# jacketsj/expANN

Measured on AMD Instinct MI355X. Metric: queries/sec at recall@10=1.0 (exact brute force), 1Mxd128 fp32, k=10, higher is better.
Workload: dtype f32; 1 GPU; brute_force_engine L2 N=1000000 d=128 fp32, 10000 batched queries, k=10 (BASELINE configs[1]); n=1000000, d=128, m=10000, k=10, metric=l2, launch=one process, one GPU, devices_visible=1, comm_ranks=0

## Files before the change

### expann_amd/csrc/expann_hip.hip

```cpp
#include "../../include/expann_hip.h"

#include <hip/hip_runtime.h>

#include <algorithm>
#include <cmath>
#include <cstdio>
#include <cstdlib>
#include <cstring>
#include <iterator>
#include <memory>
#include <mutex>
#include <string>
#include <vector>

#include "bf_append.hpp"
#include "bf_remove.hpp"
#include "bf_options.hpp"
#include "bf_plan.hpp"
#include "host_common.hpp"
#include "scan_f32.hpp"
#include "scan_gemm_bf16.hpp"
#include "scan_gemm_f16.hpp"
#include "scan_gemm_f16x.hpp"
#include "scan_gemm_f16kx.hpp"
#include "scan_direct_f16.hpp"
#include "scan_gemm_i8.hpp"
#include "scan_gemm_i8q.hpp"
#include "scan_gemm_i8w.hpp"
#include "scan_gemm_w8.hpp"
#include "scan_gemm_kl.hpp"
#include "scan_int8.hpp"
#include "scan_int8_any.hpp"
#include "filter_rows.hpp"
#include "scan_groups.hpp"
#include "append_rows.hpp"
#include "remove_rows.hpp"
#include "score_ids.hpp"
#include "select.hpp"
#include "select_range.hpp"

using namespace expann;

namespace expann {
thread_local std::string g_create_error;
}

namespace {

static_assert(kMaxK == kMaxCap / 2, "the bound on k: a candidate list holds at least 2k keys");
constexpr size_t kMaxQueriesPerPass = 32768;
constexpr int kEventPairs = 64;
constexpr uint32_t kAsyncRing = 256;
constexpr uint32_t kRingWords = 10, kRingScale = 8, kRingMark = 9;
constexpr size_t kFlagCopyBytes = sizeof(uint32_t) * 7;
constexpr uint32_t kFilterListCap = kMaxCap;

struct Level {
	uint32_t n_groups_sel;
	uint32_t group_stride;
	uint32_t classmin_blocks = 0;
	uint32_t list_rows = 0;
	uint32_t list_step = 1;
};

}


struct Config : Options {
	int dim = 0, dtype = 0, metric = 0, device = 0;
	size_t elem = 4;
	size_t q_elem = 4;
	int int_mode = -1;
	bool strict_u8 = false;
};

struct Rows {
	std::vector<unsigned char> staging;
	size_t n_staged = 0;
	MaybeOwnedPtr d_base;
	size_t n = 0;
	size_t capacity = 0;
	size_t reserved = 0;
	uint64_t id_offset = 0;
};

struct HandleDeleter {
	void operator()(expann_index* h) const { expann_destroy(h); }
};
struct U8Shadow {
	int u8_exact = 0;
	DevPtr<void> d_base_u8;
	std::unique_ptr<expann_index, HandleDeleter> u8_shadow;
};

struct F16Copy {
	DevPtr<float> d_bnmax;
	DevPtr<void> d_base_f16;
	DevPtr<float> d_bnorm_f16;
	DevPtr<float> d_bns_f16;
	float f16_scale = 0.0f;
	float f16_maxabs = 0.0f;
	size_t f16_n_pad = 0;
	size_t f16_tb = 0;
	size_t f16_rows_alloc = 0;
};
struct OtherCopies : U8Shadow {
	DevPtr<float> d_bnorm_bf;
	DevPtr<void> d_base_split;
	DevPtr<void> d_base_i8f;
	DevPtr<int> d_bp_i8f;
	DevPtr<float> d_rw_i8f;
// ... 811 lines not shown
	*tiles_big = big;
	*n_big = nb;
	*tiles_small = small;
	*n_small = ns;
	return true;
}

constexpr double kSpecFailTarget = 0.01;
double spec_fail_share(size_t k, double f, uint32_t j) {
	if (j == 0)
		return 1.0;
	if (k <= 1 || j > k - 1)
		return 0.0;
	f = std::min(1.0, std::max(0.0, f));
	const double n = (double)(k - 1);
	double term = std::pow(1.0 - f, n), below = 0.0;
	for (uint32_t i = 0; i < j; ++i) {
		below += term;
		term = f < 1.0 ? term * (n - i) / (i + 1.0) * f / (1.0 - f) : 0.0;
	}
	return f < 1.0 ? std::max(0.0, 1.0 - below) : 1.0;
}
uint32_t spec_rank_auto(size_t k, double f) {
	for (uint32_t j = 1; j < k; ++j)
		if (spec_fail_share(k, f, j) <= kSpecFailTarget)
			return j;
	return (uint32_t)k;
}
uint32_t spec_redo_slots(size_t m) {
	const size_t want = (size_t)std::ceil(4.0 * kSpecFailTarget * (double)m);
	return (uint32_t)(std::max<size_t>(1, (want + kF16TQ - 1) / kF16TQ) * kF16TQ);
}

uint32_t sample_frac_for(const expann_index* h, size_t k) {
	if (h->opt_sample_frac > 0)
		return (uint32_t)h->opt_sample_frac;
	const double expo = float_rows(h) ? 0.3 : 0.5;
	const double bytes = (double)h->n * (double)h->dim * (float_rows(h) ? 2.0 : 1.0);
	double size = (bytes >= 8 * 2.56e8 && k <= 32) ? std::min(3.0, std::pow(bytes / 2.56e8, 0.3)) : 1.0;
	if (float_rows(h) && k > 32)
		size = 0.75 * std::pow(std::max(1.0, bytes / 3.2e8), 0.25);
	const double f = 16.0 * std::pow(10.0 / (double)std::max<size_t>(1, k), expo) * size;
	return (uint32_t)std::min(48.0, std::max(4.0, std::round(f)));
}

using GemmI8qFn = void (*)(GemmI8qParams);
using SelfI8AnyFn = void (*)(const void*, uint32_t, int*, uint32_t);
using ThetaI8AnyFn = void (*)(const void*, uint32_t, const float*, int*, int*, uint32_t);
struct GemmI8qVariant {
	int d, mode;
	GemmI8qFn scan, sample;
	SelfI8Fn self;
	ThetaI8Fn theta;
	const char* name;
	int dq;
	int lds, threads, wg_per_cu;
	void (*scan_w)(GemmI8wParams) = nullptr;
	int lds_w = 0, threads_w = 0, wg_per_cu_w = 0;
	void (*sample_w)(GemmI8wParams) = nullptr;
	int tb = kF16TB;
	SelfI8AnyFn self_any = nullptr;
	ThetaI8AnyFn theta_any = nullptr;
};
#define GEMM_I8X_P(D, DQ, MODE, L2F, MN) {D, MODE, scan_gemm_w8_kernel<I8Elem, DQ, false, D, L2F>, \
	scan_gemm_w8_kernel<I8Elem, DQ, true, D, L2F>, row_self_i8_kernel<D, MODE>, query_theta_i8_kernel<D, MODE>, \
	"scan_gemm_i8x<" #DQ "," MN ">", DQ, gemm_i8q_lds_bytes<DQ>(), I8qGeom<DQ>::THREADS, I8qGeom<DQ>::WG_PER_CU}
const GemmI8qVariant kGemmI8x[] = {
    GEMM_I8X_P(768, 768, kU8L2, true, "U8L2"), GEMM_I8X_P(768, 768, kI8L2, true, "I8L2"), GEMM_I8X_P(768, 768, kI8IP, false, "I8IP"),
    GEMM_I8X_P(832, 1024, kU8L2, true, "U8L2"), GEMM_I8X_P(832, 1024, kI8L2, true, "I8L2"),
    GEMM_I8X_P(832, 1024, kI8IP, false, "I8IP"),
    GEMM_I8X_P(960, 1024, kU8L2, true, "U8L2"), GEMM_I8X_P(960, 1024, kI8L2, true, "I8L2"),
    GEMM_I8X_P(960, 1024, kI8IP, false, "I8IP"),
    GEMM_I8X_P(896, 1024, kU8L2, true, "U8L2"), GEMM_I8X_P(896, 1024, kI8L2, true, "I8L2"),
    GEMM_I8X_P(896, 1024, kI8IP, false, "I8IP")};
#undef GEMM_I8X_P
#define GEMM_I8W(D, MODE, L2F, MN) {D, MODE, nullptr, nullptr, row_self_i8_kernel<D, MODE>, \
	query_theta_i8_kernel<D, MODE>, "scan_gemm_i8w<" #D "," MN ">", D, gemm_i8q_lds_bytes<D>(), kF16Threads, \
	I8wGeom<D>::WG_PER_CU, scan_gemm_i8w_kernel<D, L2F>, gemm_i8w_lds_bytes<D>(), kF16Threads, I8wGeom<D>::WG_PER_CU, \
	scan_gemm_i8w_kernel<D, L2F, true>}
const GemmI8qVariant kGemmI8w[] = {
    GEMM_I8W(128, kU8L2, true, "U8L2"), GEMM_I8W(128, kI8L2, true, "I8L2"), GEMM_I8W(128, kI8IP, false, "I8IP"),
    GEMM_I8W(256, kU8L2, true, "U8L2"), GEMM_I8W(256, kI8L2, true, "I8L2"), GEMM_I8W(256, kI8IP, false, "I8IP")};
const GemmI8qVariant kGemmI8F = GEMM_I8W(128, kI8L2, true, "F32L2");
void (*const kGemmI8FRedo)(GemmI8wParams) = scan_gemm_i8w_kernel<128, true, false, true>;
#undef GEMM_I8W
#define GEMM_I8KL(MODE, MN) {0, MODE, nullptr, nullptr, nullptr, nullptr, "scan_gemm_i8kl<" MN ">", 0, kKlLds, kF16Threads, 1, \
	scan_gemm_kl_kernel<I8Elem, false>, kKlLds, kF16Threads, 1, scan_gemm_kl_kernel<I8Elem, true>, kKlTB, \
	row_self_i8_any_kernel<MODE>, query_theta_i8_any_kernel<MODE>}
const GemmI8qVariant kGemmI8KL[] = {GEMM_I8KL(kU8L2, "U8L2"), GEMM_I8KL(kI8L2, "I8L2"), GEMM_I8KL(kI8IP, "I8IP")};
#undef GEMM_I8KL
constexpr int kRetryGeneric = -1000;
constexpr int kStrictReject = -1001;

const GemmI8qVariant* find_gemm_i8q(ScanFamily f, int d, int mode) {
	for (const auto& v : kGemmI8w)
		if (f == ScanFamily::kI8qW && v.d == d && v.mode == mode)
			return &v;
	for (const auto& v : kGemmI8x)
		if (f == ScanFamily::kI8qX && v.d == d && v.mode == mode)
			return &v;
	for (const auto& v : kGemmI8KL)
		if (f == ScanFamily::kI8qKL && v.mode == mode)
			return &v;
	return nullptr;
}

static_assert(kI8MinRows == 2 * 256 * kF16TB, "bf_plan.hpp: two 256-tile chunks of the int8 hit-log forms");
bool plan_tables_match() {
	bool ok = kGemmF16XDbg[0].d == kF16DbgDim && kGemmI8F.d == kI8fDim;
	auto all = [&ok](const auto& tab, size_t listed, auto in) {
		size_t hits = 0;
		for (const auto& v : tab)
			hits += in(v) ? 1 : 0;
		ok = ok && hits == std::size(tab) && hits == listed;
	};
	const auto mfma_mode = [](int mode) { return mode == kU8L2 || mode == kI8L2 || mode == kI8IP; };
	all(kScanF32, 2 * count_tiles(kScanF32Tiles, std::size(kScanF32Tiles)),
	    [](const ScanVariant& v) { return has_tile(tiles_of(kScanF32Tiles, v.d), v.tq); });
	all(kScanF32Any, 2 * count_tiles(&kScanF32AnyTiles, 1), [](const ScanVariant& v) { return has_tile(&kScanF32AnyTiles, v.tq); });
	all(kScanI8, 4 * count_tiles(kScanI8Tiles, std::size(kScanI8Tiles)) + count_tiles(kScanI16Tiles, std::size(kScanI16Tiles)),
	    [](const ScanI8Variant& v) {
		    return has_tile(v.mode == kI16L2Ref ? tiles_of(kScanI16Tiles, v.d) : tiles_of(kScanI8Tiles, v.d), v.tq);
	    });
	all(kScanI8Any, 4 * count_tiles(&kScanI8AnyTiles, 1), [](const ScanI8Variant& v) { return has_tile(&kScanI8AnyTiles, v.tq); });
	all(kDirectF16, count_tiles(kDirectF16Tiles, std::size(kDirectF16Tiles)),
	    [](const DirectF16Variant& v) { return has_tile(tiles_of(kDirectF16Tiles, v.d), v.tq); });
	all(kGemmF16X, std::size(kF16XDims) + std::size(kF16YDims) + std::size(kF16KXDims), [](const GemmF16Variant& v) {
		return (has_dim(kF16XDims, v.d) && v.scan_redo) || has_dim(kF16YDims, v.d) || has_dim(kF16KXDims, v.d);
	});
	all(kGemmBf16, std::size(kBf16Dims), [](const GemmBf16Variant& v) { return has_dim(kBf16Dims, v.d); });
	all(kGemmI8, 3 * std::size(kGemmI8Dims), [&](const GemmI8Variant& v) { return has_dim(kGemmI8Dims, v.d) && mfma_mode(v.mode); });
	all(kGemmI8w, 3 * std::size(kI8qWDims), [&](const GemmI8qVariant& v) { return has_dim(kI8qWDims, v.d) && mfma_mode(v.mode); });
	all(kGemmI8x, 3 * std::size(kI8qXDims), [&](const GemmI8qVariant& v) { return has_dim(kI8qXDims, v.d) && mfma_mode(v.mode); });
	all(kGemmI8KL, 3, [&](const GemmI8qVariant& v) { return v.d == 0 && mfma_mode(v.mode); });
	return ok;
}

constexpr double kI8fClipRms = 5.5;
constexpr double kI8fTrimEnergy = 1.0 / 16.0;
constexpr double kI8fListRatio = 2.8;
constexpr double kI8fBreakEvenRatio = 3.4;
uint64_t i8f_cand_limit(const expann_index* h, size_t m, size_t k, uint32_t spec_j = 0) {
	const double rank = spec_j ? (double)spec_j : (double)k;
	return (uint64_t)(kI8fBreakEvenRatio * 1.2 * rank * sample_frac_for(h, k) * (double)m);
}

int ensure_i8f(expann_index* h, hipStream_t st) {
	if (h->i8f_state != 0)
		return EXPANN_OK;
	const size_t nv = h->n * (size_t)h->dim;
	DevBuf tmp;
	HIP_TRY(h, tmp.alloc(16));
	HIP_TRY(h, hipMemsetAsync(tmp.p, 0, 16, st));
	hipLaunchKernelGGL(i8f_stats_kernel, dim3(2048), dim3(kBlock), 0, st, (const float*)h->d_base, nv, tmp.as<double>(),
	                   reinterpret_cast<uint32_t*>(tmp.as<double>() + 1));
	unsigned char hb[16];
	float bnmax = 0.0f;
	HIP_TRY(h, hipMemcpyAsync(hb, tmp.p, 16, hipMemcpyDeviceToHost, st));
	HIP_TRY(h, hipMemcpyAsync(&bnmax, h->d_bnmax + 2, sizeof(float), hipMemcpyDeviceToHost, st));
	HIP_TRY(h, hipStreamSynchronize(st));
	double sumsq;
	float maxabs;
	std::memcpy(&sumsq, hb, 8);
	std::memcpy(&maxabs, hb + 8, 4);
	double rms = std::sqrt(sumsq / (double)nv);
	float clip = (float)std::min<double>(maxabs, kI8fClipRms * rms);
	if (maxabs > clip && std::isfinite(clip) && clip > 0.0f) {
// ... 1087 lines not shown
	sel.bn_max = h->d_bnmax ? h->d_bnmax + (gvf ? 2 : (gvb ? 1 : 0)) : nullptr;
	sel.qnrm = (use_gemm && gvf) ? h->d_qnrm : nullptr;
	if (use_i8f) {
		sel.prune_eps = 0.0f;
		sel.prune_abs = 0.0f;
		sel.row_w = h->d_rw_i8f;
		sel.q_w = h->d_i8f_q + 2 * h->i8f_q_m;
		if (h->opt_rerank_rounds != 1) {
			sel.tau_f = spec_j ? (const float*)h->d_tau_s : (const float*)h->d_tau[levels.size() & 1];
			sel.inv_2s2 = h->i8f.inv_2s2;
		}
	}
	rerank_counted = false;
	if (last && sel.rerank_base && h->opt_rerank_stats) {
		HIP_TRY(h, grow_ws(h, h->d_rerank, 16 + sizeof(uint32_t) * m));
		HIP_TRY(h, hipMemsetAsync(h->d_rerank, 0, 16 + sizeof(uint32_t) * m, st));
		sel.rerank_cnt = reinterpret_cast<uint32_t*>(h->d_rerank.as<unsigned char>() + 16);
		rerank_counted = true;
	}
	sel.overflow = h->d_overflow;
	if (last && spec_j) {
		const RedoWs ws(redo_slots, h->dim, cap);
		sel.spec_tau = h->d_tau_s;
		sel.redo_word = h->d_overflow + 3;
		sel.redo_list = reinterpret_cast<uint32_t*>(h->d_redo.as<unsigned char>() + ws.list);
		sel.redo_cap = redo_slots;
		sel.redo_bound = reinterpret_cast<float*>(h->d_redo.as<unsigned char>() + ws.bound);
	}
	const bool sum_counts = last && sel.cand_cnt && (h->profiling || use_i8f);
	if (m > 64 && sel.rerank_base && sel.cand_cnt) {
		const uint32_t sj = last ? spec_j : 0u;
		const double expect = (use_i8f ? kI8fListRatio : 1.0) * 1.2 * (sj ? (double)sj : (double)k) * sample_frac_for(h, k);
		const int rs = launch_select(h, sel, m, cap, st, select_longest_list(expect, sj), sum_counts);
		if (rs != EXPANN_OK)
			return rs;
	} else {
		if (sum_counts)
			hipLaunchKernelGGL(sum_u32_kernel, dim3(1), dim3(1024), 0, st, sel.cand_cnt, (uint32_t)m, h->d_total);
		if (m <= 64)
			sel.wave0_short = 1;
		hipLaunchKernelGGL(select_topk_fn(h, sel), dim3((uint32_t)m), dim3(kBlock), sizeof(uint64_t) * cap + 16, st, sel);
		HIP_TRY(h, hipGetLastError());
	}
	if (last && spec_j)
		return run_redo(use_i8f);
	return EXPANN_OK;
}

int SearchPass::run_redo(bool use_i8f) {
	const RedoWs ws(redo_slots, h->dim, cap);
	unsigned char* const b = h->d_redo.as<unsigned char>();
	uint32_t* const word = h->d_overflow + 3;
	const uint32_t R = redo_slots;
	RedoCompactParams cp{};
	cp.word = word;
	cp.list = reinterpret_cast<const uint32_t*>(b + ws.list);
	cp.n_slots = R;
	cp.row_bytes = (uint32_t)h->dim * 2;
	cp.q16 = h->d_q_split;
	cp.rq16 = b + ws.q16;
	cp.qnrm = h->d_qnrm;
	cp.r_qnrm = reinterpret_cast<float*>(b + ws.qnrm);
	cp.tau = h->d_tau[levels.size() & 1];
	cp.bound = h->opt_redo_bound ? reinterpret_cast<const float*>(b + ws.bound) : nullptr;
	cp.qscale = (ip && h->opt_ip_rescale) ? h->d_qscale.as<const float>() : nullptr;
	cp.eps = gemm_f16_filter_eps(h->dim);
	cp.abs_coef = std::ldexp(1.0f, -24) / h->f16_scale * std::sqrt((float)h->dim);
	cp.mul = 0.5f * h->f16_scale * h->f16_scale;
	cp.ip = ip ? 1 : 0;
	cp.r_theta = reinterpret_cast<float*>(b + ws.theta);
	cp.r_cnt = reinterpret_cast<uint32_t*>(b + ws.cnt);
	if (use_i8f) {
		cp.q8 = h->d_q8f;
		cp.rq8 = b + ws.q8;
		cp.i8_aq = h->d_i8f_q;
		cp.i8_wq_in = h->d_i8f_q + h->i8f_q_m;
		cp.r_thp = reinterpret_cast<int*>(b + ws.thp);
		cp.r_wq = reinterpret_cast<float*>(b + ws.wq);
		cp.r_tau = reinterpret_cast<float*>(b + ws.tau);
		cp.i8_inv_2s2 = h->i8f.inv_2s2;
	}
	hipLaunchKernelGGL(redo_compact_kernel, dim3(R / (kBlock / 64)), dim3(kBlock), 0, st, cp);

	const uint32_t nt = (uint32_t)((h->n + kF16TB - 1) / kF16TB);
	const uint32_t nqt = R / kF16TQ;
	const uint32_t wg_per_cu = use_i8f ? (uint32_t)kGemmI8F.wg_per_cu_w : (uint32_t)gvf->wg_per_cu;
	uint32_t chunks = pick_row_chunks(nt, 1, wg_per_cu * (uint32_t)cus, 4.0, 8, 2048, 0, nullptr);
	chunks = std::min<uint32_t>(chunks, (uint32_t)(h->log_cnt_n / (4 * (size_t)nqt)));
	if (chunks == 0 || !h->d_log)
		return h->fail(EXPANN_ERR_HIP, "redo pass: the main scan left no hit logs");
	const uint32_t tpb = (nt + chunks - 1) / chunks;
	chunks = (nt + tpb - 1) / tpb;
	const uint32_t n_logs = chunks * nqt * 4;
	const uint32_t log_cap = (uint32_t)std::min<size_t>(1u << 16, h->log_bytes / ((size_t)n_logs * 16));
	GatherLogParams gp{};
	gp.log = h->d_log.as<const uint4>();
	gp.log_cnt = h->d_log_cnt.as<const uint32_t>();
	gp.log_cap = log_cap;
	gp.n_chunks = chunks;
	gp.n_qtiles = nqt;
	gp.m = R;
	gp.cand_cnt = cp.r_cnt;
	gp.cand = reinterpret_cast<uint64_t*>(b + ws.cand);
	gp.cap = cap;
	gp.live_q = word;
	if (use_i8f) {
		GemmI8wParams wp{};
		wp.q.base = h->d_base_i8f;
		wp.q.bp = h->d_bp_i8f;
		wp.q.n_rows = (uint32_t)h->n;
		wp.q.n_tiles_sel = nt;
		wp.q.tile_stride = 1;
		wp.q.tile_run = 1;
		wp.q.tiles_per_block = tpb;
		wp.q.n_qtiles = nqt;
		wp.q.queries = cp.rq8;
		wp.q.thp = cp.r_thp;
		wp.q.m = R;
		wp.q.cand_cnt = gp.cand_cnt;
		wp.q.cand = gp.cand;
		wp.q.cap = cap;
		wp.q.live_q = word;
		wp.log = h->d_log.as<uint4>();
		wp.log_cnt = h->d_log_cnt;
		wp.log_cap = log_cap;
		wp.lost = h->d_overflow;
		hipLaunchKernelGGL(kGemmI8FRedo, dim3(chunks * nqt), dim3((uint32_t)kGemmI8F.threads_w), kGemmI8F.lds_w, st, wp);
		gp.i_thp = cp.r_thp;
		gp.i_bias = h->d_bp_i8f;
		gp.i_rw = h->d_rw_i8f;
		gp.i_mode = 3;
	} else {
		GemmF16Params fp{};
		fp.base_f16 = h->d_base_f16;
		fp.bnorm = h->bnorm_f16();
		fp.n_rows = (uint32_t)h->n;
		fp.n_tiles_sel = nt;
		fp.tile_stride = 1;
		fp.tile_run = 1;
		fp.tiles_per_block = tpb;
		fp.n_qtiles = nqt;
		fp.queries_f16 = cp.rq16;
		fp.theta = cp.r_theta;
		fp.two_inv_s2 = (ip ? 1.0f : 2.0f) / (h->f16_scale * h->f16_scale);
		fp.m = R;
		fp.cand_cnt = gp.cand_cnt;
		fp.cand = gp.cand;
		fp.cap = cap;
		fp.ksteps = (uint32_t)f16_ld(h->dim) / 32;
		fp.log = h->d_log.as<uint4>();
		fp.log_cnt = h->d_log_cnt;
		fp.log_cap = log_cap;
		fp.lost = h->d_overflow;
		fp.live_q = word;
		hipLaunchKernelGGL(gvf->scan_redo, dim3(chunks * nqt), dim3((uint32_t)gvf->threads), gvf->lds, st, fp);
		gp.theta = cp.r_theta;
		gp.key_mul = fp.two_inv_s2;
	}
	const uint32_t want = std::max<uint32_t>(1, (1024 + nqt * 4 - 1) / (nqt * 4));
	gp.chunks_per_block = std::max<uint32_t>(1, (chunks + want - 1) / want);
	gp.n_groups = (chunks + gp.chunks_per_block - 1) / gp.chunks_per_block;
	hipLaunchKernelGGL(gather_logs_kernel, dim3(nqt * 4 * gp.n_groups), dim3(kBlock), 0, st, gp);

	SelectParams sel{};
	sel.cand = gp.cand;
	sel.cand_cnt = gp.cand_cnt;
	sel.cap = cap;
	sel.k = (uint32_t)k;
	sel.id_offset = h->id_offset;
	sel.out_ids = d_ids;
	sel.out_dists = d_dists;
	sel.rerank_base = (const float*)h->d_base;
	sel.rerank_queries = (const float*)d_queries;
	sel.dim = (uint32_t)h->dim;
	sel.metric_ip = ip ? 1u : 0u;
	const float pr = ip ? 1.0f : 2.0f;
	sel.bn_max = h->d_bnmax + 2;
	sel.qnrm = cp.r_qnrm;
	if (use_i8f) {
		sel.row_w = h->d_rw_i8f;
		sel.q_w = cp.r_wq;
		if (h->opt_rerank_rounds != 1) {
			sel.tau_f = cp.r_tau;
			sel.inv_2s2 = h->i8f.inv_2s2;
		}
	} else {
		sel.prune_eps = pr * gemm_f16_filter_eps(h->dim);
		sel.prune_abs = pr * std::ldexp(1.0f, -24) / h->f16_scale * std::sqrt((float)h->dim);
	}
	sel.overflow = word;
	sel.wave0_short = 1;
	sel.slot_map = cp.list;
	sel.live_slots = word;
	sel.redo_cand = h->d_overflow + 6;
	if (rerank_counted)
		sel.rerank_cnt = reinterpret_cast<uint32_t*>(h->d_rerank.as<unsigned char>() + 16);
	hipLaunchKernelGGL(select_topk_fn(h, sel), dim3(R), dim3(kBlock), sizeof(uint64_t) * cap + 16, st, sel);
	HIP_TRY(h, hipGetLastError());
	return EXPANN_OK;
}

int SearchPass::check(int attempt, Next* next) {
	*next = kDone;
	uint64_t reranked = 0;
	if (rerank_counted) {
		unsigned long long* const total = h->d_rerank.as<unsigned long long>();
		hipLaunchKernelGGL(sum_u32_kernel, dim3(1), dim3(1024), 0, st, reinterpret_cast<const uint32_t*>(total + 2),
		                   (uint32_t)m, total);
		unsigned long long v = 0;
		HIP_TRY(h, hipMemcpyAsync(&v, total, sizeof(v), hipMemcpyDeviceToHost, st));
		HIP_TRY(h, hipStreamSynchronize(st));
		reranked = v;
	}
	if (defer_flags(h, st, attempt)) {
		h->stat_rerank_rows += reranked;
		float sc = gvf ? h->f16_scale : 0.0f;
		uint32_t* const slot = h->h_flag_ring + kRingWords * (h->async_pending - 1);
		std::memcpy(&slot[kRingScale], &sc, sizeof(float));
		if (i8f_ran && h->opt_i8_filter == 1)
			slot[kRingMark] = 0x80000000u | (uint32_t)std::min<uint64_t>(i8f_cand_limit(h, m, k, spec_j), 0x3FFFFFFFu);
		if (spec_j)
			slot[kRingMark] |= 0x40000000u;
		return EXPANN_OK;
	}
	HIP_TRY(h, hipMemcpyAsync(h->h_flags, h->d_overflow, kFlagCopyBytes, hipMemcpyDeviceToHost, st));
	HIP_TRY(h, hipStreamSynchronize(st));
	unsigned long long tot;
	std::memcpy(&tot, h->h_flags + 4, sizeof(tot));
	h->prof.candidates = tot;
	if (i8f_ran && h->opt_i8_filter == 1 && tot > i8f_cand_limit(h, m, k, spec_j))
		h->i8f_state = 2;
	if (std::getenv("EXPANN_DEBUG_LISTS")) {
		std::vector<uint32_t> cnt(m);
		HIP_TRY(h, hipMemcpy(cnt.data(), h->d_cnt, sizeof(uint32_t) * m, hipMemcpyDeviceToHost));
		std::sort(cnt.begin(), cnt.end());
		std::fprintf(stderr, "[lists] attempt %d cap %u: min %u median %u p90 %u p99 %u max %u, overflow flag %u\n", attempt, cap,
		             cnt.front(), cnt[m / 2], cnt[m * 9 / 10], cnt[m * 99 / 100], cnt.back(), h->h_flags[0]);
	}
	if (gvf) {
		float qmax;
		std::memcpy(&qmax, &h->h_flags[2], sizeof(float));
		if (!(qmax * h->f16_scale <= 60000.0f)) {
			learned.no_f16 = true;
			h->prof.retries++;
			*next = kRestart;
			return EXPANN_OK;
		}
	}
	if (h->strict_u8 && (h->h_flags[1] != 0 || h->h_flags[3] != 0))
// ... 193 lines not shown
		}
	} else {
		g_create_error = "unknown dtype";
		return EXPANN_ERR_INVALID_ARG;
	}
	if (int_mode >= 0 && dim % 64 != 0) {
		g_create_error = "8-bit rows need dim % 64 == 0 (src/distance.h:29-53, antitopo_engine.h:726)";
		return EXPANN_ERR_INVALID_ARG;
	}
	if (int_mode >= 0 && int_mode != kI16L2Ref && dim > kMaxAnyDim) {
		g_create_error = "unsupported dim " + std::to_string(dim) + ": 8-bit rows take dim <= " +
		                 std::to_string(kMaxAnyDim);
		return EXPANN_ERR_UNSUPPORTED;
	}
	int ndev = expann_device_count();
	if (ndev <= 0) {
		g_create_error = "no HIP device visible: libexpann_hip has no CPU fallback";
		return EXPANN_ERR_NO_DEVICE;
	}
	if (device < 0 || device >= ndev) {
		g_create_error = "device index out of range";
		return EXPANN_ERR_INVALID_ARG;
	}
	PlanIndex px;
	px.dtype = dtype;
	px.int_mode = int_mode;
	px.dim = dim;
	static const bool tables_match = plan_tables_match();
	if (!tables_match) {
		g_create_error = "internal: bf_plan.hpp does not list the compiled scan kernels";
		return EXPANN_ERR_UNSUPPORTED;
	}
	if (!direct_tile(px, 1)) {
		g_create_error = "unsupported dim " + std::to_string(dim) +
		                 " (built: f32 any multiple of 16 up to 4096; 8-bit any multiple of 64 up to 4096; int16 64,128)";
		return EXPANN_ERR_UNSUPPORTED;
	}
	std::unique_ptr<expann_index, HandleDeleter> h(new expann_index());
	h->dim = dim;
	h->dtype = dtype;
	h->metric = metric;
	h->device = device;
	h->elem = (dtype == EXPANN_DTYPE_F32) ? 4 : ((dtype == EXPANN_DTYPE_I16 || dtype == EXPANN_DTYPE_F16) ? 2 : 1);
	h->q_elem = (dtype == EXPANN_DTYPE_I8) ? 1 : (dtype == EXPANN_DTYPE_I16 ? 2 : 4);
	h->int_mode = int_mode;
	static_cast<Options&>(*h) = options_from_env();
	if (hipSetDevice(device) != hipSuccess || hipStreamCreate(&h->stream) != hipSuccess) {
		g_create_error = "hipSetDevice/hipStreamCreate failed";
		return EXPANN_ERR_HIP;
	}
	struct LdsNeed {
		const void* fn;
		int bytes;
		const char* label;
	};
	std::vector<LdsNeed> needs;
	const int sel_lds = (int)(sizeof(uint64_t) * kMaxCap + 16);
	needs.push_back({(const void*)select_topk_kernel<float>, sel_lds, "select_topk_kernel"});
	needs.push_back({(const void*)select_topk_kernel<_Float16>, sel_lds, "select_topk_kernel"});
	needs.push_back({(const void*)select_topk_kernel<float, true>, sel_lds, "select_topk_kernel"});
	for (const auto& v : kGemmF16X)
		if (v.d == dim) {
			needs.push_back({(const void*)v.scan, v.lds, "scan_gemm_f16x_kernel"});
			needs.push_back({(const void*)v.sample, v.lds, "scan_gemm_f16x_kernel"});
			if (v.scan_redo)
				needs.push_back({(const void*)v.scan_redo, v.lds, "scan_gemm_f16x_kernel"});
		}
	if ((dtype == EXPANN_DTYPE_F32 || dtype == EXPANN_DTYPE_F16) && f16kl_dim(dim)) {
		needs.push_back({(const void*)kGemmF16KL.scan, kGemmF16KL.lds, "scan_gemm_kl_kernel, fp16"});
		needs.push_back({(const void*)kGemmF16KL.sample, kGemmF16KL.lds, "scan_gemm_kl_kernel, fp16"});
	}
	if (kGemmF16XDbg[0].d == dim)
		needs.push_back({(const void*)kGemmF16XDbg[0].scan, kGemmF16XDbg[0].lds, "scan_gemm_f16x_kernel"});
	for (const auto& v : kGemmI8x)
		if (v.d == dim) {
			needs.push_back({(const void*)v.scan, v.lds, "scan_gemm_w8_kernel, int8"});
			needs.push_back({(const void*)v.sample, v.lds, "scan_gemm_w8_kernel, int8"});
		}
	for (const auto& v : kGemmI8w)
		if (v.d == dim) {
			needs.push_back({(const void*)v.scan_w, v.lds_w, "scan_gemm_i8w_kernel"});
			needs.push_back({(const void*)v.sample_w, v.lds_w, "scan_gemm_i8w_kernel"});
		}
	if (dim == kGemmI8F.d)
		needs.push_back({(const void*)kGemmI8FRedo, kGemmI8F.lds_w, "scan_gemm_i8w_kernel, redo instance"});
	if (any_dim_i8(dim, int_mode))
		for (const auto& v : kGemmI8KL)
			if (v.mode == int_mode) {
				needs.push_back({(const void*)v.scan_w, v.lds_w, "scan_gemm_kl_kernel, int8"});
				needs.push_back({(const void*)v.sample_w, v.lds_w, "scan_gemm_kl_kernel, int8"});
			}
	for (const auto& v : kGemmBf16)
		if (v.d == dim)
			needs.push_back({(const void*)v.scan, 2 * kGemmTB * dim * (int)sizeof(float), "scan_gemm_bf16x3_kernel"});
	for (const auto& v : kGemmI8)
		if (v.d == dim && v.mode == int_mode)
			needs.push_back({(const void*)v.scan, 2 * gemm_i8_tb(dim) * dim, "scan_gemm_i8_kernel"});
	for (const LdsNeed& need : needs)
		if (hipFuncSetAttribute(need.fn, hipFuncAttributeMaxDynamicSharedMemorySize, need.bytes) != hipSuccess) {
			g_create_error = std::string("hipFuncSetAttribute(") + need.label + ") failed";
			return EXPANN_ERR_HIP;
		}
	*out = h.release();
	return EXPANN_OK;
}

void expann_destroy(expann_index* h) {
	if (!h)
		return;
	hipSetDevice(h->device);
	if (h->stream) hipStreamSynchronize(h->stream);
	if (h->side_stream) hipStreamSynchronize(h->side_stream);
	delete h;
}

const char* expann_last_error(const expann_index* h) {
	return h ? h->err.c_str() : g_create_error.c_str();
}

int expann_add(expann_index* h, const void* rows, size_t n) {
	if (!h)
		return EXPANN_ERR_INVALID_ARG;
	if (!rows && n)
		return h->fail(EXPANN_ERR_INVALID_ARG, "rows == NULL");
	if (h->d_base)
		return h->fail(EXPANN_ERR_INVALID_ARG, "index already built");
	const size_t bytes = n * (size_t)h->dim * h->elem;
	const unsigned char* src = static_cast<const unsigned char*>(rows);
	h->staging.insert(h->staging.end(), src, src + bytes);
	h->n_staged += n;
	return EXPANN_OK;
}

int expann_build(expann_index* h) {
	if (!h)
		return EXPANN_ERR_INVALID_ARG;
	if (h->d_base)
		return h->fail(EXPANN_ERR_INVALID_ARG, "index already built");
	if (h->n_staged == 0)
		return h->fail(EXPANN_ERR_INVALID_ARG, "build() on an empty index");
	if (h->n_staged >= (1ull << 32) - 32)
		return h->fail(EXPANN_ERR_UNSUPPORTED, "more than 2^32 rows per shard");
	HIP_TRY(h, hipSetDevice(h->device));
	drop_row_filter(h);
	drop_row_groups(h);
	void* rows = nullptr;
	const size_t capacity = std::max(h->n_staged, h->reserved);
	HIP_TRY(h, hipMalloc(&rows, capacity * (size_t)h->dim * h->elem));
	h->d_base.own(rows);
	h->capacity = capacity;
	HIP_TRY(h, hipMemcpy(h->d_base, h->staging.data(), h->staging.size(), hipMemcpyHostToDevice));
	h->n = h->n_staged;
	std::vector<unsigned char>().swap(h->staging);
	if (f16_copy_at_build(plan_index(h)))
		return ensure_f16(h, find_f16(f16_geometry(h->dim), h->dim), h->stream);
	return EXPANN_OK;
}

int expann_set_base_device(expann_index* h, const void* d_rows, size_t n, uint64_t id_offset) {
	if (!h)
		return EXPANN_ERR_INVALID_ARG;
	if (!d_rows || n == 0)
		return h->fail(EXPANN_ERR_INVALID_ARG, "empty device base");
	if (n >= (1ull << 32) - 32)
		return h->fail(EXPANN_ERR_UNSUPPORTED, "more than 2^32 rows per shard");
	h->forget<RowCopies>();
	drop_row_filter(h);
	drop_row_groups(h);
// ... 1665 lines not shown
```

### expann_amd/csrc/scan_gemm_i8w.hpp

```cpp
#pragma once
#include "scan_gemm_i8q.hpp"

namespace expann {

template <int D> struct I8wGeom {
	static constexpr int WG_PER_CU = D == 128 ? 3 : 2;
	static constexpr int QCAP = D == 128 ? 64 : kF16WaveQueue;
};
template <int D> constexpr int gemm_i8w_lds_bytes() {
	return kF16Bufs * (kF16TB * D + kF16Waves * 256) + kF16Waves * I8wGeom<D>::QCAP * kF16EntryBytes + kF16TQ * 4 + 64;
}
static_assert(gemm_i8w_lds_bytes<128>() * 3 <= 160 * 1024 && gemm_i8w_lds_bytes<256>() * 2 <= 160 * 1024,
              "LDS budget per CU");

template <int D, bool L2FORM, bool SAMPLE = false, bool REDO = false>
__global__ __launch_bounds__(kF16Threads, I8wGeom<D>::WG_PER_CU) void scan_gemm_i8w_kernel(GemmI8wParams pw) {
	static_assert(D == 128 || D == 256, "built for d = 128, 256");
	const GemmI8qParams& p = pw.q;
	constexpr int THREADS = kF16Threads, WAVES = kF16Waves, WGQ = kF16TQ, QCAP = I8wGeom<D>::QCAP;
	constexpr int ROWB = D, CH = ROWB / 16;
	constexpr int KS = D / 64;
	constexpr int TILE_BYTES = kF16TB * ROWB;
	constexpr int RPB = (ROWB < 256) ? 256 / ROWB : 1;
	constexpr int SWM = (CH < 16 ? CH : 16) - 1;
	constexpr int NBUF = kF16Bufs;
	constexpr int kNever = -2147483647 - 1;
	extern __shared__ __attribute__((aligned(16))) unsigned char smem[];

	const int tid = threadIdx.x;
	const int lane = tid & 63;
	const int wave = __builtin_amdgcn_readfirstlane(tid >> 6);
	const int l15 = lane & 15, lq = lane >> 4;
	uint32_t qtile = blockIdx.x % p.n_qtiles;
	uint32_t chunk = blockIdx.x / p.n_qtiles;
	if (p.xcd_map) {
		const uint32_t j = blockIdx.x >> 3;
		qtile = j % p.n_qtiles;
		chunk = (blockIdx.x & 7) + 8 * (j / p.n_qtiles);
	}
	const uint32_t wg_q0 = qtile * WGQ;
	if (!SAMPLE && p.live_q && wg_q0 >= (*p.live_q & kRedoCountMask))
		return;
	const uint32_t q0 = wg_q0 + wave * 64;

	const uint32_t t0 = chunk * p.tiles_per_block;
	uint32_t t1 = t0 + p.tiles_per_block;
	if (t1 > p.n_tiles_sel)
		t1 = p.n_tiles_sel;
	uint32_t* const my_log_cnt = SAMPLE ? nullptr : pw.log_cnt + (size_t)blockIdx.x * WAVES + wave;
	if (t0 >= t1) {
		if (SAMPLE) {
			for (uint32_t i = lane; i < 64 * 32; i += 64)
				if (q0 + (i >> 5) < p.m)
					p.sample_out[((size_t)(q0 + (i >> 5)) * p.n_chunks + chunk) * 32 + (i & 31)] = kNever;
		} else if (lane == 0) {
			*my_log_cnt = 0;
		}
		return;
	}

	unsigned char* const bn_slots = smem + NBUF * TILE_BYTES;
	struct QEntry {
		int acc[16];
		int bp;
		uint32_t row;
		uint32_t qrow0;
		uint32_t pad;
	};
	static_assert(sizeof(QEntry) == kF16EntryBytes, "queue entry size");
	QEntry* const queue = reinterpret_cast<QEntry*>(bn_slots + NBUF * WAVES * 256) + wave * QCAP;
	uint32_t* const fills = reinterpret_cast<uint32_t*>(bn_slots + NBUF * WAVES * 256 + WAVES * QCAP * kF16EntryBytes) + WGQ;

	i32x4 a[4][KS];
#pragma unroll
	for (int tq = 0; tq < 4; ++tq) {
		uint32_t qi = q0 + tq * 16 + l15;
		if (qi >= p.m)
			qi = p.m - 1;
		const i32x4* src = reinterpret_cast<const i32x4*>((const unsigned char*)p.queries + (size_t)qi * ROWB);
#pragma unroll
		for (int s = 0; s < KS; ++s)
			a[tq][s] = src[4 * s + lq];
	}
	i32x4 th[4];
#pragma unroll
	for (int tq = 0; tq < 4; ++tq)
#pragma unroll
		for (int r = 0; r < 4; ++r) {
			const uint32_t qi = q0 + tq * 16 + 4 * lq + r;
			th[tq][r] = (qi < p.m && !SAMPLE) ? p.thp[qi] : kNever / 2;
		}
#pragma unroll
	for (int tq = 0; tq < 4; ++tq) {
#pragma unroll
		for (int s = 0; s < KS; ++s)
			asm volatile("" : "+v"(a[tq][s]));
		asm volatile("" : "+v"(th[tq]));
	}
// ... 20 lines not shown
		if (i < N_STAGE) {
			unsigned char* dst0 = smem + buf * TILE_BYTES + wave * 64 * 16;
			__builtin_amdgcn_global_load_lds((const __attribute__((address_space(1))) void*)(tb + soff[i < N_STAGE ? i : 0]),
			                                 (__attribute__((address_space(3))) void*)(dst0 + i * THREADS * 16), 16, 0, 0);
		} else {
			__builtin_amdgcn_global_load_lds((const __attribute__((address_space(1))) void*)(p.bp + row0 + lane),
			                                 (__attribute__((address_space(3))) void*)(bn_slots + (buf * WAVES + wave) * 256),
			                                 4, 0, 0);
		}
	};
	auto stage_src = [&](uint32_t t, uint32_t& row0) -> const unsigned char* {
		if (t > t1 - 1)
			t = t1 - 1;
		row0 = tile_row0(t);
		return (const unsigned char*)p.base + (size_t)row0 * ROWB;
	};
	auto stage = [&](uint32_t t, int buf) {
		uint32_t row0;
		const unsigned char* tb = stage_src(t, row0);
#pragma unroll
		for (int i = 0; i < LOADS; ++i)
			stage_piece(tb, row0, buf, i);
	};

	uint32_t wfill = 0;
	uint32_t glog_n = 0;
	uint4* const my_log = SAMPLE ? nullptr : pw.log + ((size_t)blockIdx.x * WAVES + wave) * pw.log_cap;
	auto flush_own = [&]() {
		const uint32_t n = wfill < (uint32_t)QCAP ? wfill : (uint32_t)QCAP;
		for (uint32_t base = 0; base < n * 16; base += 128) {
			bool hit[2];
			int cv[2];
			uint32_t row[2], qi[2];
#pragma unroll
			for (int u = 0; u < 2; ++u) {
				const uint32_t i = base + 64 * u + lane;
				const QEntry& e = queue[i < n * 16 ? i >> 4 : 0];
				const uint32_t v = i & 15;
				cv[u] = e.acc[v];
				row[u] = e.row;
				hit[u] = i < n * 16 && cv[u] >= e.bp && row[u] < p.n_rows;
				qi[u] = e.qrow0 + 16 * (v >> 2) + (v & 3);
			}
#pragma unroll
			for (int u = 0; u < 2; ++u) {
				const unsigned long long mask = __builtin_amdgcn_ballot_w64(hit[u]);
				if (mask == 0)
					continue;
				const uint32_t pos = glog_n + __builtin_amdgcn_mbcnt_hi((uint32_t)(mask >> 32),
				                                                        __builtin_amdgcn_mbcnt_lo((uint32_t)mask, 0u));
				if (hit[u] && pos < pw.log_cap)
					my_log[pos] = make_uint4((uint32_t)cv[u], row[u], qi[u], (uint32_t)queue[(base + 64 * u + lane) >> 4].bp);
				glog_n += (uint32_t)__builtin_popcountll(mask);
			}
		}
		wfill = 0;
	};
	auto push_hits = [&](const i32x4 (&acc)[4][4], int tc, unsigned long long mask, bool mine, int bp,
	                     uint32_t row0) {
		static_assert(QCAP >= 64, "a tile column's hits fit an empty queue");
		if (wfill + (uint32_t)__builtin_popcountll(mask) > (uint32_t)QCAP)
			flush_own();
		uint32_t qrow0 = q0 + 4 * lq;
		asm volatile("" : "+v"(qrow0));
		const uint32_t brow = row0 + tc * 16 + l15;
		const uint32_t slot = wfill + __builtin_amdgcn_mbcnt_hi((uint32_t)(mask >> 32),
		                                                        __builtin_amdgcn_mbcnt_lo((uint32_t)mask, 0u));
		if (mine) {
			if (slot < (uint32_t)QCAP) {
				QEntry& e = queue[slot];
#pragma unroll
				for (int tq = 0; tq < 4; ++tq)
#pragma unroll
					for (int r = 0; r < 4; ++r)
						e.acc[tq * 4 + r] = acc[tq][tc][r];
				e.bp = bp;
				e.row = brow;
				e.qrow0 = qrow0;
			}
		}
		wfill += (uint32_t)__builtin_popcountll(mask);
	};

	const bool idle = REDO && p.live_q && q0 >= (*p.live_q & kRedoCountMask);
	if (REDO && idle && lane == 0)
		fills[wave] = 0;
	stage(t0, 0);
	stage(t0 + 1, 1);
	asm volatile("s_waitcnt vmcnt(0) lgkmcnt(0)\n\ts_barrier" ::: "memory");
	if (REDO && idle) {
		int ibuf = 0;
		for (uint32_t t = t0; t < t1; ++t) {
			const int pbuf = ibuf == 0 ? NBUF - 1 : ibuf - 1;
			asm volatile("" ::: "memory");
			__builtin_amdgcn_s_waitcnt(0x0070);
			__builtin_amdgcn_s_barrier();
			asm volatile("" ::: "memory");
			stage(t + 2, pbuf);
			ibuf = ibuf + 1 == NBUF ? 0 : ibuf + 1;
		}
		if (lane == 0)
			*my_log_cnt = 0;
		asm volatile("s_waitcnt vmcnt(0)" ::: "memory");
		return;
	}

	i32x4 acc[4][4];
	int buf = 0;
	uint32_t since_look = 0;
	auto frag_at = [&](int b, int tc, int s) -> i32x4 {
		return *reinterpret_cast<const i32x4*>(smem + ((uint32_t)b * TILE_BYTES + aoff[s]) + tc * 16 * ROWB);
	};
	auto read_bp = [&](int (&bp)[4], int b) {
		const int* slot = reinterpret_cast<const int*>(bn_slots + (b * WAVES + wave) * 256);
#pragma unroll
		for (int tc = 0; tc < 4; ++tc)
			bp[tc] = slot[tc * 16 + l15];
	};
	auto col_max = [&](int pc) -> int {
		int m0 = max3i(acc[0][pc][0], acc[0][pc][1], acc[0][pc][2]);
		int m1 = max3i(acc[0][pc][3], acc[1][pc][0], acc[1][pc][1]);
		int m2 = max3i(acc[1][pc][2], acc[1][pc][3], acc[2][pc][0]);
		int m3 = max3i(acc[2][pc][1], acc[2][pc][2], acc[2][pc][3]);
		int m4 = max3i(acc[3][pc][0], acc[3][pc][1], acc[3][pc][2]);
		m0 = max3i(m0, m1, acc[3][pc][3]);
		m2 = max3i(m2, m3, m4);
		return max(m0, m2);
	};
	int bpv[4];
	i32x4 smax[2][4];
#pragma unroll
	for (int par = 0; par < 2; ++par)
#pragma unroll
		for (int tq = 0; tq < 4; ++tq)
			smax[par][tq] = i32x4{kNever, kNever, kNever, kNever};
	auto fold = [&](int par) {
#pragma unroll
		for (int tq = 0; tq < 4; ++tq)
#pragma unroll
			for (int r = 0; r < 4; ++r)
				smax[par][tq][r] = max3i(smax[par][tq][r], acc[tq][par][r], acc[tq][par + 2][r]);
	};
	auto mfma_part = [&](int tc, const i32x4 (&f)[KS], int s0, int s1) {
		const int nb = -bpv[tc];
		const i32x4 c0 = {nb, nb, nb, nb};
#pragma unroll
		for (int s = s0; s < s1; ++s)
#pragma unroll
			for (int tq = 0; tq < 4; ++tq)
				acc[tq][tc] = __builtin_amdgcn_mfma_i32_16x16x64_i8(a[tq][s], f[s], s == 0 ? (SAMPLE ? c0 : th[tq]) : acc[tq][tc], 0, 0, 0);
	};

	i32x4 fb[2][KS];
#pragma unroll
	for (int s = 0; s < KS; ++s)
		fb[0][s] = frag_at(0, 0, s);
	read_bp(bpv, 0);
	__builtin_amdgcn_s_waitcnt(0xC07F);
	for (uint32_t t = t0; t < t1; ++t) {
		const int nbuf = buf + 1 == NBUF ? 0 : buf + 1;
		const int pbuf = buf == 0 ? NBUF - 1 : buf - 1;
		int gmax[4];
		int bpn[4];
		__builtin_amdgcn_s_setprio(1);
		mfma_part(0, fb[0], 0, 1);
		__builtin_amdgcn_sched_barrier(0);
#pragma unroll
		for (int s = 0; s < KS; ++s)
			fb[1][s] = frag_at(buf, 1, s);
		__builtin_amdgcn_sched_barrier(0);
		mfma_part(0, fb[0], 1, KS);
		__builtin_amdgcn_sched_barrier(0);
		mfma_part(1, fb[1], 0, 1);
		__builtin_amdgcn_sched_barrier(0);
#pragma unroll
		for (int s = 0; s < KS; ++s)
			fb[0][s] = frag_at(buf, 2, s);
		__builtin_amdgcn_sched_barrier(0);
		mfma_part(1, fb[1], 1, KS);
		if (!SAMPLE) {
			gmax[0] = col_max(0);
			asm volatile("" : "+v"(gmax[0]));
		}
		__builtin_amdgcn_sched_barrier(0);
		__builtin_amdgcn_s_setprio(0);
		const bool look = !SAMPLE && ++since_look == kF16FlushEvery;
		if (look && lane == 0)
			fills[wave] = wfill;
// ... 89 lines not shown
```

Measured before the change: 7.550 million queries/s.

## Replace i8f redo GEMM-plus-log-gather with a streaming per-wave redo kernel

For the int8 fallback redo pass, the tiled GEMM scan kernel (REDO instance) and the separate gather_logs kernel are replaced by a new redo_stream_i8 kernel. Each wave streams a range of 16-row base columns straight from global memory with register double-buffering, runs MFMA against the live redo queries, and appends hits directly into candidate lists with atomics. This drops the LDS staging, the hit-log buffer and one kernel launch, and it handles only the live query count instead of full query tiles. In exchange, concurrent atomicAdd contention on cand_cnt can rise. Without LDS, each wave also reloads its query fragments for every 64-query group.

```diff
diff --git a/expann_amd/csrc/expann_hip.hip b/expann_amd/csrc/expann_hip.hip
--- a/expann_amd/csrc/expann_hip.hip
+++ b/expann_amd/csrc/expann_hip.hip
@@ -27,6 +27,7 @@
 #include "scan_gemm_i8.hpp"
 #include "scan_gemm_i8q.hpp"
 #include "scan_gemm_i8w.hpp"
+#include "scan_redo_i8.hpp"
 #include "scan_gemm_w8.hpp"
 #include "scan_gemm_kl.hpp"
 #include "scan_int8.hpp"
@@ -1004,7 +1005,6 @@
     GEMM_I8W(128, kU8L2, true, "U8L2"), GEMM_I8W(128, kI8L2, true, "I8L2"), GEMM_I8W(128, kI8IP, false, "I8IP"),
     GEMM_I8W(256, kU8L2, true, "U8L2"), GEMM_I8W(256, kI8L2, true, "I8L2"), GEMM_I8W(256, kI8IP, false, "I8IP")};
 const GemmI8qVariant kGemmI8F = GEMM_I8W(128, kI8L2, true, "F32L2");
-void (*const kGemmI8FRedo)(GemmI8wParams) = scan_gemm_i8w_kernel<128, true, false, true>;
 #undef GEMM_I8W
 #define GEMM_I8KL(MODE, MN) {0, MODE, nullptr, nullptr, nullptr, nullptr, "scan_gemm_i8kl<" MN ">", 0, kKlLds, kF16Threads, 1, \
 	scan_gemm_kl_kernel<I8Elem, false>, kKlLds, kF16Threads, 1, scan_gemm_kl_kernel<I8Elem, true>, kKlTB, \
@@ -2258,55 +2258,47 @@
 	}
 	hipLaunchKernelGGL(redo_compact_kernel, dim3(R / (kBlock / 64)), dim3(kBlock), 0, st, cp);
 
-	const uint32_t nt = (uint32_t)((h->n + kF16TB - 1) / kF16TB);
-	const uint32_t nqt = R / kF16TQ;
-	const uint32_t wg_per_cu = use_i8f ? (uint32_t)kGemmI8F.wg_per_cu_w : (uint32_t)gvf->wg_per_cu;
-	uint32_t chunks = pick_row_chunks(nt, 1, wg_per_cu * (uint32_t)cus, 4.0, 8, 2048, 0, nullptr);
-	chunks = std::min<uint32_t>(chunks, (uint32_t)(h->log_cnt_n / (4 * (size_t)nqt)));
-	if (chunks == 0 || !h->d_log)
-		return h->fail(EXPANN_ERR_HIP, "redo pass: the main scan left no hit logs");
-	const uint32_t tpb = (nt + chunks - 1) / chunks;
-	chunks = (nt + tpb - 1) / tpb;
-	const uint32_t n_logs = chunks * nqt * 4;
-	const uint32_t log_cap = (uint32_t)std::min<size_t>(1u << 16, h->log_bytes / ((size_t)n_logs * 16));
-	GatherLogParams gp{};
-	gp.log = h->d_log.as<const uint4>();
-	gp.log_cnt = h->d_log_cnt.as<const uint32_t>();
-	gp.log_cap = log_cap;
-	gp.n_chunks = chunks;
-	gp.n_qtiles = nqt;
-	gp.m = R;
-	gp.cand_cnt = cp.r_cnt;
-	gp.cand = reinterpret_cast<uint64_t*>(b + ws.cand);
-	gp.cap = cap;
-	gp.live_q = word;
+	uint32_t* const r_cnt = cp.r_cnt;
+	uint64_t* const r_cand = reinterpret_cast<uint64_t*>(b + ws.cand);
 	if (use_i8f) {
-		GemmI8wParams wp{};
-		wp.q.base = h->d_base_i8f;
-		wp.q.bp = h->d_bp_i8f;
-		wp.q.n_rows = (uint32_t)h->n;
-		wp.q.n_tiles_sel = nt;
-		wp.q.tile_stride = 1;
-		wp.q.tile_run = 1;
-		wp.q.tiles_per_block = tpb;
-		wp.q.n_qtiles = nqt;
-		wp.q.queries = cp.rq8;
-		wp.q.thp = cp.r_thp;
-		wp.q.m = R;
-		wp.q.cand_cnt = gp.cand_cnt;
-		wp.q.cand = gp.cand;
-		wp.q.cap = cap;
-		wp.q.live_q = word;
-		wp.log = h->d_log.as<uint4>();
-		wp.log_cnt = h->d_log_cnt;
-		wp.log_cap = log_cap;
-		wp.lost = h->d_overflow;
-		hipLaunchKernelGGL(kGemmI8FRedo, dim3(chunks * nqt), dim3((uint32_t)kGemmI8F.threads_w), kGemmI8F.lds_w, st, wp);
-		gp.i_thp = cp.r_thp;
-		gp.i_bias = h->d_bp_i8f;
-		gp.i_rw = h->d_rw_i8f;
-		gp.i_mode = 3;
+		RedoStreamParams rp{};
+		rp.base = h->d_base_i8f;
+		rp.bp = h->d_bp_i8f;
+		rp.n_rows = (uint32_t)h->n;
+		rp.n_cols = (uint32_t)((h->n + kF16TB - 1) / kF16TB) * (kF16TB / 16);
+		const uint32_t n_waves = (uint32_t)cus * kRedoStreamWavesPerCu;
+		rp.cols_per_wave = (rp.n_cols + n_waves - 1) / n_waves;
+		rp.cols_per_wave = (rp.cols_per_wave + kRedoStreamU - 1) / kRedoStreamU * kRedoStreamU;
+		rp.queries = cp.rq8;
+		rp.thp = cp.r_thp;
+		rp.n_slots = R;
+		rp.live_q = word;
+		rp.cand_cnt = r_cnt;
+		rp.cand = r_cand;
+		rp.cap = cap;
+		hipLaunchKernelGGL(redo_stream_i8_kernel, dim3(n_waves / kRedoStreamWaves), dim3(kRedoStreamThreads), 0, st, rp);
 	} else {
+		const uint32_t nt = (uint32_t)((h->n + kF16TB - 1) / kF16TB);
+		const uint32_t nqt = R / kF16TQ;
+		uint32_t chunks = pick_row_chunks(nt, 1, (uint32_t)gvf->wg_per_cu * (uint32_t)cus, 4.0, 8, 2048, 0, nullptr);
+		chunks = std::min<uint32_t>(chunks, (uint32_t)(h->log_cnt_n / (4 * (size_t)nqt)));
+		if (chunks == 0 || !h->d_log)
+			return h->fail(EXPANN_ERR_HIP, "redo pass: the main scan left no hit logs");
+		const uint32_t tpb = (nt + chunks - 1) / chunks;
+		chunks = (nt + tpb - 1) / tpb;
+		const uint32_t n_logs = chunks * nqt * 4;
+		const uint32_t log_cap = (uint32_t)std::min<size_t>(1u << 16, h->log_bytes / ((size_t)n_logs * 16));
+		GatherLogParams gp{};
+		gp.log = h->d_log.as<const uint4>();
+		gp.log_cnt = h->d_log_cnt.as<const uint32_t>();
+		gp.log_cap = log_cap;
+		gp.n_chunks = chunks;
+		gp.n_qtiles = nqt;
+		gp.m = R;
+		gp.cand_cnt = r_cnt;
+		gp.cand = r_cand;
+		gp.cap = cap;
+		gp.live_q = word;
 		GemmF16Params fp{};
 		fp.base_f16 = h->d_base_f16;
 		fp.bnorm = h->bnorm_f16();
@@ -2332,15 +2324,15 @@
 		hipLaunchKernelGGL(gvf->scan_redo, dim3(chunks * nqt), dim3((uint32_t)gvf->threads), gvf->lds, st, fp);
 		gp.theta = cp.r_theta;
 		gp.key_mul = fp.two_inv_s2;
-	}
-	const uint32_t want = std::max<uint32_t>(1, (1024 + nqt * 4 - 1) / (nqt * 4));
-	gp.chunks_per_block = std::max<uint32_t>(1, (chunks + want - 1) / want);
-	gp.n_groups = (chunks + gp.chunks_per_block - 1) / gp.chunks_per_block;
-	hipLaunchKernelGGL(gather_logs_kernel, dim3(nqt * 4 * gp.n_groups), dim3(kBlock), 0, st, gp);
+		const uint32_t want = std::max<uint32_t>(1, (1024 + nqt * 4 - 1) / (nqt * 4));
+		gp.chunks_per_block = std::max<uint32_t>(1, (chunks + want - 1) / want);
+		gp.n_groups = (chunks + gp.chunks_per_block - 1) / gp.chunks_per_block;
+		hipLaunchKernelGGL(gather_logs_kernel, dim3(nqt * 4 * gp.n_groups), dim3(kBlock), 0, st, gp);
+	}
 
 	SelectParams sel{};
-	sel.cand = gp.cand;
-	sel.cand_cnt = gp.cand_cnt;
+	sel.cand = r_cand;
+	sel.cand_cnt = r_cnt;
 	sel.cap = cap;
 	sel.k = (uint32_t)k;
 	sel.id_offset = h->id_offset;
@@ -2700,8 +2692,6 @@
 			needs.push_back({(const void*)v.scan_w, v.lds_w, "scan_gemm_i8w_kernel"});
 			needs.push_back({(const void*)v.sample_w, v.lds_w, "scan_gemm_i8w_kernel"});
 		}
-	if (dim == kGemmI8F.d)
-		needs.push_back({(const void*)kGemmI8FRedo, kGemmI8F.lds_w, "scan_gemm_i8w_kernel, redo instance"});
 	if (any_dim_i8(dim, int_mode))
 		for (const auto& v : kGemmI8KL)
 			if (v.mode == int_mode) {
diff --git a/expann_amd/csrc/scan_gemm_i8w.hpp b/expann_amd/csrc/scan_gemm_i8w.hpp
--- a/expann_amd/csrc/scan_gemm_i8w.hpp
+++ b/expann_amd/csrc/scan_gemm_i8w.hpp
@@ -13,7 +13,7 @@
 static_assert(gemm_i8w_lds_bytes<128>() * 3 <= 160 * 1024 && gemm_i8w_lds_bytes<256>() * 2 <= 160 * 1024,
               "LDS budget per CU");
 
-template <int D, bool L2FORM, bool SAMPLE = false, bool REDO = false>
+template <int D, bool L2FORM, bool SAMPLE = false>
 __global__ __launch_bounds__(kF16Threads, I8wGeom<D>::WG_PER_CU) void scan_gemm_i8w_kernel(GemmI8wParams pw) {
 	static_assert(D == 128 || D == 256, "built for d = 128, 256");
 	const GemmI8qParams& p = pw.q;
@@ -200,28 +200,9 @@
 		wfill += (uint32_t)__builtin_popcountll(mask);
 	};
 
-	const bool idle = REDO && p.live_q && q0 >= (*p.live_q & kRedoCountMask);
-	if (REDO && idle && lane == 0)
-		fills[wave] = 0;
 	stage(t0, 0);
 	stage(t0 + 1, 1);
 	asm volatile("s_waitcnt vmcnt(0) lgkmcnt(0)\n\ts_barrier" ::: "memory");
-	if (REDO && idle) {
-		int ibuf = 0;
-		for (uint32_t t = t0; t < t1; ++t) {
-			const int pbuf = ibuf == 0 ? NBUF - 1 : ibuf - 1;
-			asm volatile("" ::: "memory");
-			__builtin_amdgcn_s_waitcnt(0x0070);
-			__builtin_amdgcn_s_barrier();
-			asm volatile("" ::: "memory");
-			stage(t + 2, pbuf);
-			ibuf = ibuf + 1 == NBUF ? 0 : ibuf + 1;
-		}
-		if (lane == 0)
-			*my_log_cnt = 0;
-		asm volatile("s_waitcnt vmcnt(0)" ::: "memory");
-		return;
-	}
 
 	i32x4 acc[4][4];
 	int buf = 0;
diff --git a/expann_amd/csrc/scan_redo_i8.hpp b/expann_amd/csrc/scan_redo_i8.hpp
--- /dev/null
+++ b/expann_amd/csrc/scan_redo_i8.hpp
@@ -0,0 +1,120 @@
+#pragma once
+#include "scan_gemm_i8q.hpp"
+
+namespace expann {
+
+constexpr int kRedoStreamThreads = 256;
+constexpr int kRedoStreamWaves = kRedoStreamThreads / 64;
+constexpr int kRedoStreamU = 2;
+constexpr int kRedoStreamWavesPerCu = 16;
+
+struct RedoStreamParams {
+	const void* base;
+	const int* bp;
+	uint32_t n_rows;
+	uint32_t n_cols;
+	uint32_t cols_per_wave;
+	const void* queries;
+	const int* thp;
+	uint32_t n_slots;
+	const uint32_t* live_q;
+	uint32_t* cand_cnt;
+	uint64_t* cand;
+	uint32_t cap;
+};
+
+__global__ __launch_bounds__(kRedoStreamThreads, 4) void redo_stream_i8_kernel(RedoStreamParams p) {
+	constexpr int U = kRedoStreamU, ROWB = 128, KS = 2;
+	const int lane = threadIdx.x & 63;
+	const int l15 = lane & 15, lq = lane >> 4;
+	const uint32_t wave = __builtin_amdgcn_readfirstlane(blockIdx.x * kRedoStreamWaves + (threadIdx.x >> 6));
+	const uint32_t c0 = wave * p.cols_per_wave;
+	uint32_t c1 = c0 + p.cols_per_wave;
+	if (c1 > p.n_cols)
+		c1 = p.n_cols;
+	uint32_t live = *p.live_q & kRedoCountMask;
+	if (live > p.n_slots)
+		live = p.n_slots;
+	if (c0 >= c1 || live == 0)
+		return;
+
+	struct Col {
+		i32x4 b[KS];
+		int bp;
+	};
+	const unsigned char* const lane_rows = (const unsigned char*)p.base + l15 * ROWB + lq * 16;
+	auto load = [&](Col (&f)[U], uint32_t c) {
+#pragma unroll
+		for (int u = 0; u < U; ++u) {
+			const uint32_t cc = c + u < c1 ? c + u : c1 - 1;
+			const unsigned char* src = lane_rows + (size_t)cc * (16 * ROWB);
+#pragma unroll
+			for (int s = 0; s < KS; ++s)
+				f[u].b[s] = *reinterpret_cast<const i32x4*>(src + 64 * s);
+			f[u].bp = p.bp[cc * 16 + l15];
+		}
+	};
+
+	for (uint32_t q0 = 0; q0 < live; q0 += 64) {
+		const uint32_t groups = (live - q0 + 15) / 16;
+		i32x4 a[4][KS], th[4];
+#pragma unroll
+		for (int tq = 0; tq < 4; ++tq) {
+			const i32x4* src = reinterpret_cast<const i32x4*>((const unsigned char*)p.queries + (size_t)(q0 + tq * 16 + l15) * ROWB);
+#pragma unroll
+			for (int s = 0; s < KS; ++s)
+				a[tq][s] = src[4 * s + lq];
+#pragma unroll
+			for (int r = 0; r < 4; ++r)
+				th[tq][r] = p.thp[q0 + tq * 16 + 4 * lq + r];
+		}
+		auto column = [&](const Col& f, uint32_t c) {
+			const uint32_t row = c * 16 + l15;
+			const bool row_ok = row < p.n_rows;
+#pragma unroll
+			for (int tq = 0; tq < 4; ++tq) {
+				if ((uint32_t)tq >= groups)
+					break;
+				i32x4 acc = __builtin_amdgcn_mfma_i32_16x16x64_i8(a[tq][0], f.b[0], th[tq], 0, 0, 0);
+				acc = __builtin_amdgcn_mfma_i32_16x16x64_i8(a[tq][1], f.b[1], acc, 0, 0, 0);
+				const int top = max(max(acc[0], acc[1]), max(acc[2], acc[3]));
+				if (__builtin_amdgcn_ballot_w64(top >= f.bp && row_ok) == 0)
+					continue;
+				uint32_t qlane = q0 + 4 * lq;
+				asm volatile("" : "+v"(qlane));
+#pragma unroll
+				for (int r = 0; r < 4; ++r)
+					if (acc[r] >= f.bp && row_ok) {
+						const uint32_t qi = qlane + tq * 16 + r;
+						const uint32_t slot = atomicAdd(&p.cand_cnt[qi], 1u);
+						if (slot < p.cap) {
+							const float kappa = (float)(f.bp - acc[r]);
+							p.cand[(size_t)qi * p.cap + slot] =
+							    make_key(f.bp > kI8fBpMin && f.bp < kI8fBpMax ? kappa : -__builtin_inff(), row);
+						}
+					}
+			}
+		};
+
+		auto columns = [&](const Col (&f)[U], uint32_t c) {
+#pragma unroll
+			for (int u = 0; u < U; ++u)
+				if (c + u < c1)
+					column(f[u], c + u);
+		};
+		Col f0[U], f1[U];
+		load(f0, c0);
+		for (uint32_t c = c0;; c += 2 * U) {
+			load(f1, c + U);
+			columns(f0, c);
+			if (c + U >= c1)
+				break;
+			load(f0, c + 2 * U);
+			columns(f1, c + U);
+			if (c + 2 * U >= c1)
+				break;
+		}
+	}
+}
+
+}
```

Result: faster. 7.705 million queries/s (median of 6 runs) (+2.1%).
